# aask1357/hilcodec

Hardware: AMD Instinct MI355X
Metric: audio-seconds/sec (xRT) encode+RVQ+decode, 24 kHz batch=256 (higher is better)
Workload: dtype f32

## Files before the change

### hilcodec_amd/csrc/resblock_kernel.h

```cpp
#pragma once
#include "resblock_gemm.h"
#include "stream_gemm.h"

namespace {

struct Cols {
  long b;
  int t;
  int t_in;
  unsigned boff;
  unsigned hoff;
  int head, tail;
};
static_assert(sizeof(Cols) == 32, "no padding");

template <int C, bool STREAM, bool SCARRY = false, int NB = 1, bool W8 = false, int DRU = 0, bool POST = false, bool SPEC0 = false>
__global__ __launch_bounds__((Cfg<C, STREAM, SCARRY, NB, W8, DRU, POST, SPEC0>::NT), (Cfg<C, STREAM, SCARRY, NB, W8, DRU, POST, SPEC0>::MINW)) void resblock_kernel(ResArgs a) {
  using K = Cfg<C, STREAM, SCARRY, NB, W8, DRU, POST, SPEC0>;
  constexpr int DR = K::DR, UR = K::UR;
  using Pipe = WeightPipe<K>;
  constexpr int CBW = K::CBW, NW = K::NW, NT = K::NT, RW = K::RW, RB = K::RB, XS = K::XS, TO = K::TO, RSTEP = K::RSTEP;
  __shared__ __attribute__((aligned(16))) float Xbuf[4 + C * XS];
  constexpr bool DW_RELOAD = NB > 1 && K::NARROW && (4 + C * XS + NB * C * DWS) * 4 > 156 * 1024;
  __shared__ __attribute__((aligned(16))) float DW[(DW_RELOAD ? 1 : NB) * C * DWS];
  constexpr bool DWIDE = DR == 5 || DR == 8;
  __shared__ __attribute__((aligned(16))) float DWD[(DR > 0 && !DWIDE) ? 2 * C * DDS : 4];
  __shared__ __attribute__((aligned(16))) float HS[(STREAM && !K::NARROW) ? 2 * C * 4 : 4];
  __shared__ __attribute__((aligned(16))) float PR[POST ? POST_CLASSES * K::NCOL : 4];
  static_assert(!POST || (K::RPI * K::NW == POST_CLASSES), "a row class of the closing conv = the rows one half-wave walks");
  __shared__ __attribute__((aligned(16))) float SEG[SPEC0 ? (STREAM ? 256 : 192) : 4];
  __shared__ __attribute__((aligned(16))) float SEGS[SPEC0 ? (STREAM ? 256 : 192) : 4];
  float* const X = Xbuf + 4;
  const int tid = threadIdx.x, lane = tid & 63;
  const int wave = __builtin_amdgcn_readfirstlane(tid >> 6);
  constexpr int NCB = K::NCOL / 32;
  const int colblk = wave % NCB;
  const int wclass = wave / NCB;
  const int rowblk0 = wclass * CBW;
#if defined(HILC_DEBUG_WAVE_STAMPS)
  constexpr int WS_MAXB = 48;
  unsigned long long* ws_base = nullptr;
  int ws_k = 0;
#define STAMP(i) do { } while (0)
#define lds_barrier() do {                                                                                          \
    const unsigned long long t0_ = __builtin_amdgcn_s_memtime();                                                   \
    asm volatile("s_waitcnt lgkmcnt(0)" ::: "memory");                                                             \
    const unsigned long long t1_ = __builtin_amdgcn_s_memtime();                                                   \
    asm volatile("s_waitcnt lgkmcnt(0)\n\ts_barrier" ::: "memory");                                                 \
    const unsigned long long t2_ = __builtin_amdgcn_s_memtime();                                                   \
    if (ws_base != nullptr && lane == 0 && ws_k < WS_MAXB - 1) {                                                   \
      ws_base[ws_k * 3] = t0_; ws_base[ws_k * 3 + 1] = t1_; ws_base[ws_k * 3 + 2] = t2_;                           \
    }                                                                                                              \
    ++ws_k;                                                                                                        \
  } while (0)
#elif defined(HILC_DEBUG_STAMPS)
#define STAMP(i) do { if (a.dbg && tid == 0) a.dbg[stamp_tile * 8 + (i)] = __builtin_amdgcn_s_memtime(); } while (0)
  long stamp_tile = blockIdx.x;
#else
#define STAMP(i) do { } while (0)
#endif
  const int T = a.T;
  const int nblk = NB == 1 ? 1 : a.nblk;
  auto load_taps = [&](const ResBlk& bq, float* dst) {
    if constexpr (DW_RELOAD && !STREAM) {
      constexpr int NE = C * DWS;
      static_assert(NE % NT == 0, "whole rounds");
#pragma unroll
      for (int i = 0; i < NE / NT; ++i) {
        const int e = tid + i * NT;
        const int m = e / DWS, j = e - m * DWS;
        const float* src = j < 5 ? bq.dw1_w + (m * 5 + j) : (j == 5 ? bq.dw1_b + m : (j < 11 ? bq.dw2_w + (m * 5 + (j - 6)) : bq.dw2_b + m));
        dst[e] = *src;
      }
    } else if constexpr (DW_RELOAD) {
      constexpr int NE = C * DWS;
      static_assert(NE % NT == 0, "whole rounds");
#pragma unroll 3
      for (int i = 0; i < NE / NT; ++i) {
        const int e = tid + i * NT;
        const int m = e / DWS, j = e - m * DWS;
        const float* src = j < 5 ? bq.dw1_w + (m * 5 + j) : (j == 5 ? bq.dw1_b + m : (j < 11 ? bq.dw2_w + (m * 5 + (j - 6)) : bq.dw2_b + m));
        dst[e] = *src;
      }
    }
  };
  if constexpr (!DW_RELOAD) {
    constexpr int RND = (C + NT - 1) / NT;
    if constexpr (NB == 1 && STREAM) {
      const ResBlk& bq = a.blk[0];
#pragma unroll
      for (int it = 0; it < RND; ++it) {
        const int m = tid + it * NT;
        const int mc = (C % NT == 0 || m < C) ? m : C - 1;
#pragma unroll
        for (int w4 = 0; w4 < DWS / 4; ++w4) {
          float t4[4];
#pragma unroll
          for (int e = 0; e < 4; ++e) {
            const int j = 4 * w4 + e;
            t4[e] = j < 5 ? bq.dw1_w[mc * 5 + j] : (j == 5 ? bq.dw1_b[mc] : (j < 11 ? bq.dw2_w[mc * 5 + (j - 6)] : bq.dw2_b[mc]));
          }
          if (C % NT == 0 || m < C) *reinterpret_cast<f32x4*>(&DW[m * DWS + 4 * w4]) = f32x4{t4[0], t4[1], t4[2], t4[3]};
          __builtin_amdgcn_sched_barrier(0);
        }
      }
    } else {
    float tv[NB][RND][DWS];
#pragma unroll
    for (int q = 0; q < NB; ++q) {
      if (q < nblk) {
        const ResBlk& bq = a.blk[q];
#pragma unroll
        for (int it = 0; it < RND; ++it) {
          const int m = tid + it * NT;
          const int mc = (C % NT == 0 || m < C) ? m : C - 1;
#pragma unroll
          for (int j = 0; j < 5; ++j) tv[q][it][j] = bq.dw1_w[mc * 5 + j];
          tv[q][it][5] = bq.dw1_b[mc];
#pragma unroll
          for (int j = 0; j < 5; ++j) tv[q][it][6 + j] = bq.dw2_w[mc * 5 + j];
          tv[q][it][11] = bq.dw2_b[mc];
        }
      }
    }
#pragma unroll
    for (int q = 0; q < NB; ++q) {
      if (q < nblk) {
#pragma unroll
        for (int it = 0; it < RND; ++it) {
          const int m = tid + it * NT;
          if (C % NT == 0 || m < C) {
#pragma unroll
            for (int w4 = 0; w4 < DWS / 4; ++w4)
              *reinterpret_cast<f32x4*>(&DW[(q * C + m) * DWS + 4 * w4]) =
                  f32x4{tv[q][it][4 * w4], tv[q][it][4 * w4 + 1], tv[q][it][4 * w4 + 2], tv[q][it][4 * w4 + 3]};
          }
        }
      }
    }
    }
  }
  if constexpr (DR > 0 && !DWIDE) {
    constexpr int RND = (2 * C + NT - 1) / NT;
    float tw[RND][2 * DR + 1];
#pragma unroll
    for (int it = 0; it < RND; ++it) {
      const int m = tid + it * NT;
      const int mc = ((2 * C) % NT == 0 || m < 2 * C) ? m : 2 * C - 1;
#pragma unroll
      for (int j = 0; j < 2 * DR; ++j) tw[it][j] = a.dn.dw_w[mc * 2 * DR + j];
      tw[it][2 * DR] = a.dn.dw_b[mc];
    }
#pragma unroll
    for (int it = 0; it < RND; ++it) {
      const int m = tid + it * NT;
      if ((2 * C) % NT == 0 || m < 2 * C) {
#pragma unroll
        for (int j = 0; j < DDS; ++j) DWD[m * DDS + j] = j < 2 * DR ? tw[it][j] : (j == 8 ? tw[it][2 * DR] : 0.f);
      }
    }
  }
  if (tid < 4) Xbuf[tid] = 0.f;
  const int rsub = wave * K::RPI + (K::RPI > 1 ? lane / (K::NCOL / 4) : 0);
  const int c4 = (lane & (K::NCOL / 4 - 1)) * 4;
  [[maybe_unused]] const unsigned row_b = (unsigned)T * 4u;
  [[maybe_unused]] const bool one_head = STREAM && !K::NARROW && T >= K::NCOL;

  auto columns_of = [&](long tile) -> Cols {
    Cols s;
    s.boff = 0; s.hoff = 0; s.head = false; s.tail = false;
    if constexpr (STREAM) {
      const int flat = (int)tile * TO - K::HALO + c4;
      s.t_in = flat >= 0 && flat < a.B * T;
      const unsigned ub = s.t_in ? __umulhi((unsigned)flat, a.div_magic) >> a.div_shift : 0u;
      s.b = ub;
      s.t = s.t_in ? flat - (int)ub * T : 0;
      s.boff = (ub * (unsigned)(C * T) + (unsigned)s.t) * 4u;
      s.hoff = ub * (unsigned)(C * 4);
      s.head = s.t_in && s.t == 0;
      s.tail = s.t_in && c4 >= K::HALO && s.t == T - 4;
    } else {
      s.b = tile / a.tiles;
      s.t = (int)(tile - s.b * a.tiles) * TO + c4;
      s.t_in = s.t >= 0 && s.t < T;
    }
    return s;
  };
  auto xrow = [&](const Cols& s, int m) -> const f32x4* {
    if constexpr (STREAM)
      return reinterpret_cast<const f32x4*>(reinterpret_cast<const char*>(a.x) + (s.boff + (unsigned)m * row_b));
    else
      return reinterpret_cast<const f32x4*>(a.x + s.b * (long)C * T + (long)m * T + (s.t_in ? s.t : 0));
  };
  auto yrow = [&](const Cols& s, int m) -> f32x4* {
    if constexpr (STREAM)
      return reinterpret_cast<f32x4*>(reinterpret_cast<char*>(a.y) + (s.boff + (unsigned)m * row_b));
    else
      return reinterpret_cast<f32x4*>(a.y + s.b * (long)C * T + (long)m * T + s.t);
  };

  [[maybe_unused]] const float* hb0 = a.x;
  [[maybe_unused]] const float* hb1 = a.x;
  [[maybe_unused]] bool hv0 = false, hv1 = false;
  [[maybe_unused]] int blk_off = 0;
  Cols cs;
  const bool lane0 = c4 == 0, lane_last = c4 == K::NCOL - 4;
  auto prev_base = [&](int which) -> lptr_t {
    if constexpr (!K::CARRYMODE) return (lptr_t)(X + rsub * XS + c4 - 4);
    else return lane0 ? (lptr_t)(X + rsub * XS + K::NCOL + which * 4 + blk_off) : (lptr_t)(X + rsub * XS + c4 - 4);
  };
  auto prevs_of = [&](lptr_t pb, int m0, int which, f32x4 (&prev)[K::RB]) {
    if constexpr (!STREAM) {
#pragma unroll
      for (int i = 0; i < K::RB; ++i) prev[i] = *(lvec_t)(pb + i * RSTEP * XS);
    } else {
      bool staged = false;
      if constexpr (!K::NARROW) staged = one_head;
      if (staged) {
#pragma unroll
        for (int i = 0; i < K::RB; ++i) {
          const lptr_t pa = cs.head ? (lptr_t)(HS + (which * C + m0 + RSTEP * i) * 4) : pb + i * RSTEP * XS;
          prev[i] = *(lvec_t)pa;
        }
      } else {
        f32x4 hv[K::RB];
#pragma unroll
        for (int i = 0; i < K::RB; ++i)
          hv[i] = *reinterpret_cast<const f32x4*>((which ? hb1 : hb0) + ((which ? hv1 : hv0) ? cs.hoff + (unsigned)(m0 + RSTEP * i) * 4u : 0u));
#pragma unroll
        for (int i = 0; i < K::RB; ++i) {
          const f32x4 own = *(lvec_t)(pb + i * RSTEP * XS);
#pragma unroll
          for (int e = 0; e < 4; ++e) prev[i][e] = cs.head ? ((which ? hv1 : hv0) ? hv[i][e] : 0.f) : own[e];
        }
      }
    }
  };
  auto carry_out = [&](lptr_t xp, int which, const f32x4 (&cur)[K::RB]) {
    if constexpr (K::CARRYMODE) {
      if (lane_last) {
#pragma unroll
        for (int i = 0; i < K::RB; ++i) *(lvec_t)(xp + i * RSTEP * XS + 4 + which * 4 + blk_off) = cur[i];
      }
    }
  };

  float touch = 0.f;
  constexpr int LPR = K::NCOL / 32;
#ifdef HILC_RES_NO_UTOUCH
  constexpr bool UTOUCH = false;
#else
  constexpr bool UTOUCH = !STREAM && UR > 0 && !K::NARROW && (K::NCOL / (UR > 0 ? UR : 1)) % 32 == 0;
#endif
  constexpr int LPRU = UTOUCH ? K::NCOL / UR / 32 : 1;
  constexpr int NTOUCH = STREAM ? 1 : (UTOUCH ? (2 * C * LPRU + NT - 1) / NT : (C * LPR + NT - 1) / NT);
  float tv[NTOUCH];
#pragma unroll
  for (int i = 0; i < NTOUCH; ++i) tv[i] = 0.f;
  __shared__ long s_next;
  long run0 = blockIdx.x, run1 = a.total_tiles;
  long tile = blockIdx.x;
  if constexpr (K::CARRYMODE) {
    if (a.classes > 1) {
      const unsigned P = gridDim.x / (unsigned)a.classes, u = blockIdx.x % P, c = blockIdx.x / P;
      const long s0 = (long)u * a.total_tiles / P, len = (long)(u + 1) * a.total_tiles / P - s0;
      run0 = s0 + ((len * (long)a.cum[c]) >> 16);
      run1 = s0 + ((len * (long)a.cum[c + 1]) >> 16);
    } else if (a.run_tiles > 0) {
      run0 = (long)blockIdx.x * a.run_tiles;
      run1 = run0 + a.run_tiles < a.total_tiles ? run0 + a.run_tiles : a.total_tiles;
    } else {
      run0 = (long)blockIdx.x * a.total_tiles / gridDim.x;
      run1 = ((long)blockIdx.x + 1) * a.total_tiles / gridDim.x;
    }
    const bool mid = STREAM ? (run0 * TO) % T != 0 : run0 % a.tiles != 0;
    tile = (mid && run0 < run1) ? run0 - 1 : run0;
  }
  cs = columns_of(tile < run1 ? tile : 0);
  f32x4 xr[RW];
  if (UR == 0 && !SPEC0 && tile < run1) {
#pragma unroll
    for (int i = 0; i < RW; ++i) xr[i] = *xrow(cs, rsub + RSTEP * i);
  }
  lds_barrier();
  while (tile < run1) {
    const bool warm = K::CARRYMODE && tile < run0;
    constexpr bool TICKETS = !K::CARRYMODE && K::NW == 4;
    if constexpr (K::CARRYMODE && !STREAM) {
      if (tile % a.tiles == 0) {
        constexpr int NSLOT = 2 * NB + K::DCAR / 2 + (POST ? 1 : 0);
        for (int e = tid; e < NSLOT * C; e += NT)
          *reinterpret_cast<f32x4*>(X + (e / NSLOT) * XS + K::NCOL + (e % NSLOT) * 4) = f32x4{0.f, 0.f, 0.f, 0.f};
      }
    }
    if constexpr (!K::CARRYMODE) {
      if (TICKETS && a.sched != nullptr && tid == 0) s_next = (long)gridDim.x + atomicAdd(a.sched, 1);
    }
#if defined(HILC_DEBUG_WAVE_STAMPS)
    if (a.dbg != nullptr) {
      if (ws_base != nullptr && lane == 0) ws_base[(WS_MAXB - 1) * 3 + 1] = (unsigned long long)ws_k;
      ws_base = a.dbg + ((tile * NW + wave) * (long)WS_MAXB) * 3;
      if (lane == 0) { ws_base[(WS_MAXB - 1) * 3] = blockIdx.x; ws_base[(WS_MAXB - 1) * 3 + 2] = __builtin_amdgcn_s_memtime(); }
    }
    ws_k = 0;
#elif defined(HILC_DEBUG_STAMPS)
    stamp_tile = tile;
#endif
    STAMP(0);
    long next_tile = K::CARRYMODE ? tile + 1 : tile + gridDim.x;
    if constexpr (UR > 0) {
      const ResUp& up = a.up;
      const int Tin = T / UR;
      const int q0 = cs.t / UR, p0 = cs.t - q0 * UR;
      f32x16 acc[CBW];
#pragma unroll
      for (int i = 0; i < CBW; ++i)
#pragma unroll
        for (int r = 0; r < 16; ++r) acc[i][r] = 0.f;
#pragma nounroll
      for (int h = 0; h < 2; ++h) {
        const float* wu = (h ? up.w_hi : up.w_lo) + (long)wclass * (C * C / K::RH);
        asm volatile("" : "+s"(wu));
        {
          constexpr int UB = RW % 6 == 0 ? 6 : RB;
          constexpr bool UEXP = UR == 5;
          lptr_t xp = (lptr_t)(X + rsub * XS + c4);
          const bool has_prev = cs.t_in && q0 >= 1;
          [[maybe_unused]] const bool has_next = cs.t_in && q0 + 1 < Tin;
#pragma unroll
          for (int i0 = 0; i0 < RW; i0 += UB) {
            float xc[UB], xq[UB];
            [[maybe_unused]] float xn[UB];
            f32x4 wa[UB];
            [[maybe_unused]] f32x4 wb[UB];
#pragma unroll
            for (int i = 0; i < UB; ++i) {
              const int k = h * C + rsub + RSTEP * (i0 + i);
              const long row = (long)cs.b * (2 * C) + k;
              const float* xi = up.xin + (cs.t_in ? row * Tin + q0 : 0);
              xc[i] = xi[0];
              const float* pp = has_prev ? xi - 1 : (up.hist != nullptr && cs.t_in ? up.hist + row : xi);
              xq[i] = pp[0];
              if constexpr (UR == 2) {
                xn[i] = xi[cs.t_in ? 1 : 0];
                wa[i] = *reinterpret_cast<const f32x4*>(up.tr_w + k * 4);
              } else if constexpr (UEXP) {
                xn[i] = xi[has_next ? 1 : 0];
                const float* tw = up.tr_w + ((long)k * UR + p0) * 8;
                wa[i] = *reinterpret_cast<const f32x4*>(tw);
                wb[i] = *reinterpret_cast<const f32x4*>(tw + 4);
              } else {
                wa[i] = *reinterpret_cast<const f32x4*>(up.tr_w + k * (2 * UR) + p0);
                wb[i] = *reinterpret_cast<const f32x4*>(up.tr_w + k * (2 * UR) + UR + p0);
              }
            }
#pragma unroll
            for (int i = 0; i < UB; ++i) {
              const float a1 = prologue(xc[i], up.in_scale, 1);
              const float a0 = has_prev ? prologue(xq[i], up.in_scale, 1) : (up.hist != nullptr ? xq[i] : 0.f);
              f32x4 u;
              float a_last = a1;
              if constexpr (UR == 2) {
                const float a2 = prologue(xn[i], up.in_scale, 1);
                u[0] = fmaf(wa[i].x, a1, wa[i].z * a0);
                u[1] = fmaf(wa[i].y, a1, wa[i].w * a0);
                u[2] = fmaf(wa[i].x, a2, wa[i].z * a1);
                u[3] = fmaf(wa[i].y, a2, wa[i].w * a1);
                a_last = a2;
              } else if constexpr (UEXP) {
                const float a2 = has_next ? prologue(xn[i], up.in_scale, 1) : 0.f;
#pragma unroll
                for (int e = 0; e < 4; ++e) {
                  const bool nx = p0 + e >= UR;
                  u[e] = fmaf(wa[i][e], nx ? a2 : a1, wb[i][e] * (nx ? a1 : a0));
                }
                a_last = p0 + 3 >= UR ? a2 : a1;
              } else {
#pragma unroll
                for (int e = 0; e < 4; ++e) u[e] = fmaf(wa[i][e], a1, wb[i][e] * a0);
              }
              *(lvec_t)(xp + i * RSTEP * XS) = zero_unless(cs.t_in, u);
              if constexpr (STREAM) {
                if (cs.tail && !warm && up.hist_out != nullptr)
                  up.hist_out[(long)cs.b * (2 * C) + h * C + rsub + RSTEP * (i0 + i)] = a_last;
              }
            }
            xp += UB * RSTEP * XS;
            asm volatile("" : "+v"(xp));
            __builtin_amdgcn_sched_barrier(0);
          }
        }
        Pipe wp;
        wp.prefetch(wu, lane);
        lds_barrier();
        if constexpr (K::NARROW) gemm_phase_rolled<K, false>(wu, X, acc, wp, colblk, lane);
        else gemm_phase<K, false>(wu, X, acc, wp, colblk, lane);
        lds_barrier();
      }
      acc_to_x<K>(acc, X, rowblk0, colblk, lane);
      lds_barrier();
      {
        lptr_t xp = (lptr_t)(X + rsub * XS + c4);
#pragma unroll
        for (int i = 0; i < RW; ++i) {
          const float bv = up.bias != nullptr ? up.bias[rsub + RSTEP * i] : 0.f;
          f32x4 v = *(lvec_t)(xp + i * RSTEP * XS);
#pragma unroll
          for (int e = 0; e < 4; ++e) v[e] = up.bias != nullptr ? __fadd_rn(v[e], bv) : v[e];
          xr[i] = v;
        }
      }
      lds_barrier();
    }
    if constexpr (SPEC0) {
      const ResSpec0& sp = a.spec;
      constexpr int N = 64, NBIN = 33, SROWS = 40, KP0 = 4, DEPTH0 = 2;
      [[maybe_unused]] int split = K::NCOL;
      if constexpr (STREAM) {
        const int F0 = (int)tile * TO;
        const unsigned bA = __umulhi((unsigned)F0, a.div_magic) >> a.div_shift;
        const int tA0 = F0 - (int)bA * T;
        const int nxt = T - tA0;
        split = nxt < K::NCOL ? nxt : K::NCOL;
        const int lenA = (N - 1) + split;
        for (int i = tid; i < 2 * (N - 1) + K::NCOL; i += NT) {
          const bool second = i >= lenA;
          const unsigned b = bA + (second ? 1u : 0u);
          const int t = second ? i - lenA - (N - 1) : tA0 - (N - 1) + i;
          float v = 0.f;
          if (b < (unsigned)a.B) {
            if (t >= 0) v = sp.wav[(long)b * T + t];
            else if (sp.hist != nullptr && t >= -sp.hist_len) v = sp.hist[(long)b * sp.hist_len + sp.hist_len + t];
          }
          SEG[i] = v;
          SEGS[i] = v * sp.pre_in_scale;
        }
        for (int i = tid; i < (SROWS - NBIN) * 128; i += NT) X[(NBIN + (i >> 7)) * XS + (i & 127)] = 0.f;
      } else {
      const int f0 = cs.t - c4;
      {
        const int s0 = f0 - (N - 1);
        const float* wb = sp.wav + cs.b * (long)T;
        for (int i = tid; i < 127 + N; i += NT) {
          const int t = s0 + i;
          const float v = (t >= 0 && t < T) ? wb[t] : 0.f;
          SEG[i] = v;
          SEGS[i] = v * sp.pre_in_scale;
        }
        for (int i = tid; i < (SROWS - NBIN) * 128; i += NT) X[(NBIN + (i >> 7)) * XS + (i & 127)] = 0.f;
      }
      }
      lds_barrier();
      const int kh = lane >> 5, col = colblk * 32 + (lane & 31);
      const int colx = col + ((STREAM && col >= split) ? N - 1 : 0);
      f32x16 acc[CBW];
      {
        int off[8];
#pragma unroll
        for (int p = 0; p < 8; ++p) off[p] = colx + 2 * p + kh;
        auto bop = [&](int P) -> float { return SEG[off[P & 7] + 16 * (P >> 3)]; };
        stream_gemm<CBW, KP0, DEPTH0, N / 2 / KP0>(sp.dft, acc, lane, bop);
      }
      float nyq_im = 0.f;
#pragma unroll 8
      for (int k = 0; k < N; ++k) nyq_im = fmaf(sp.nyq[k], SEG[colx + k], nyq_im);
      const SpecFinish finish = SpecFinish::make(sp.mean, sp.stdv, sp.normalize);
#pragma unroll
      for (int i = 0; i < CBW; ++i) {
#pragma unroll
        for (int r = 0; r < 16; r += 2) {
          const int row = i * 32 + acc_row(r, lane);
          if (i == 0 && r == 0) {
            if (kh == 0) {
              X[0 * XS + col] = finish(acc[0][0], 0.f);
              X[(N / 2) * XS + col] = finish(acc[0][1], nyq_im);
            } else {
              X[(row >> 1) * XS + col] = finish(acc[0][0], acc[0][1]);
            }
          } else {
            X[(row >> 1) * XS + col] = finish(acc[i][r], acc[i][r + 1]);
          }
        }
      }
      lds_barrier();
      {
        const float* sl = X + kh * XS + col;
        auto bop = [&](int P) -> float { return sl[2 * P * XS]; };
        stream_gemm<CBW, KP0, DEPTH0, SROWS / 2 / KP0>(sp.pw, acc, lane, bop);
      }
      lds_barrier();
      acc_to_x<K>(acc, X, rowblk0, colblk, lane);
      lds_barrier();
      {
        lptr_t xp = (lptr_t)(X + rsub * XS + c4);
        float sm[8];
        const int c4x = c4 + ((STREAM && c4 >= split) ? N - 1 : 0);
#pragma unroll
        for (int j = 0; j < 8; ++j) sm[j] = SEGS[c4x + j + N - 5];
#pragma unroll
        for (int i = 0; i < RW; ++i) {
          const int m = rsub + RSTEP * i;
          const float bv = sp.bias != nullptr ? sp.bias[m] : 0.f;
          const float pb = sp.pre_b != nullptr ? sp.pre_b[m] : 0.f;
          float w5[5];
#pragma unroll
          for (int j = 0; j < 5; ++j) w5[j] = sp.pre_w[m * 5 + j];
          f32x4 v = *(lvec_t)(xp + i * RSTEP * XS);
#pragma unroll
          for (int e = 0; e < 4; ++e) {
            float acc5 = 0.f;
#pragma unroll
            for (int j = 0; j < 5; ++j) acc5 = fmaf(w5[j], sm[e + j], acc5);
            const float rr = sp.pre_b != nullptr ? __fadd_rn(acc5, pb) : acc5;
            float t = v[e];
            if (sp.bias != nullptr) t = __fadd_rn(t, bv);
            t = __fmul_rn(t, sp.out_scale);
            v[e] = __fadd_rn(t, rr);
          }
          xr[i] = v;
          if (i % 2 == 1) __builtin_amdgcn_sched_barrier(0);
        }
      }
      lds_barrier();
    }
#pragma nounroll
    for (int blk = 0; blk < nblk; ++blk) {
    const ResBlk& bp = a.blk[NB == 1 ? 0 : blk];
    const bool final_blk = NB == 1 || blk == nblk - 1;
    const bool last_blk = DR == 0 && !POST && final_blk;
    [[maybe_unused]] const bool post_blk = POST && final_blk;
    Cols cn = cs;
    bool have_next = false;
    if constexpr (NB > 1) blk_off = 8 * blk;
    const float* const DWb = DW + ((NB == 1 || DW_RELOAD) ? 0 : blk * C * DWS);
    if constexpr (DW_RELOAD) load_taps(bp, DW);
    if constexpr (STREAM) {
      hb0 = bp.hist1 != nullptr ? bp.hist1 : a.x;
      hb1 = bp.hist2 != nullptr ? bp.hist2 : a.x;
      hv0 = bp.hist1 != nullptr;
      hv1 = bp.hist2 != nullptr;
    }
    const float* w1t = bp.w1t + (long)wclass * (C * C / K::RH);
    const float* w2t = bp.w2t + (long)wclass * (C * C / K::RH);
    asm volatile("" : "+s"(w1t), "+s"(w2t));
    [[maybe_unused]] f32x4 hstage[(STREAM && !K::NARROW) ? (2 * C + NT - 1) / NT : 1];
    [[maybe_unused]] bool stage_hs = false;
    if constexpr (STREAM && !K::NARROW) {
      if (one_head) {
        const int first = (int)tile * TO - K::HALO, last = first + K::NCOL - 1;
        const unsigned bh = __umulhi((unsigned)last, a.div_magic) >> a.div_shift;
        const int hcol = (int)bh * T;
        stage_hs = hcol >= first && (int)bh < a.B;
        if (stage_hs) {
#pragma unroll
          for (int q = 0; q < (2 * C + NT - 1) / NT; ++q) {
            const int e = tid + q * NT;
            const int which = e >= C ? 1 : 0, m = e - which * C;
            f32x4 v = {0.f, 0.f, 0.f, 0.f};
            if (e < 2 * C && (which ? hv1 : hv0)) v = *reinterpret_cast<const f32x4*>((which ? hb1 : hb0) + bh * (unsigned)(C * 4) + (unsigned)m * 4u);
            hstage[q] = v;
          }
        }
      }
    }
    Pipe wp;
    wp.prefetch(w1t, lane);
    {
      lptr_t xp = (lptr_t)(X + rsub * XS + c4);
#pragma unroll
      for (int i0 = 0; i0 < RW; i0 += RB) {
#pragma unroll
        for (int i = 0; i < RB; ++i)
          *(lvec_t)(xp + i * RSTEP * XS) = prologue4v(zero_unless(cs.t_in, xr[i0 + i]), bp.pre_scale, 1);
        xp += RB * RSTEP * XS;
        asm volatile("" : "+v"(xp));
      }
    }
#pragma unroll
    for (int i = 0; i < NTOUCH; ++i) touch += tv[i];
    if constexpr (STREAM && !K::NARROW) {
      if (stage_hs) {
#pragma unroll
        for (int q = 0; q < (2 * C + NT - 1) / NT; ++q) {
          const int e = tid + q * NT;
          if (e < 2 * C) *reinterpret_cast<f32x4*>(&HS[e * 4]) = hstage[q];
        }
      }
    }
    lds_barrier();
    STAMP(1);
    if (TICKETS && a.sched != nullptr) next_tile = s_next;

    f32x16 acc[CBW];
    if constexpr (K::NARROW) gemm_phase_rolled<K>(w1t, X, acc, wp, colblk, lane);
    else gemm_phase<K>(w1t, X, acc, wp, colblk, lane);
    lds_barrier();
    STAMP(2);
    acc_to_x<K>(acc, X, rowblk0, colblk, lane);
    lds_barrier();
    STAMP(3);

    wp.prefetch(w2t, lane);
    lptr_t xp3 = (lptr_t)(X + rsub * XS + c4);
    lptr_t pb3 = prev_base(0);
#pragma unroll
    for (int i0 = 0; i0 < RW; i0 += RB) {
      f32x4 cur[RB], prev[RB], wa[RB];
      f32x2 wb[RB];
#pragma unroll
      for (int i = 0; i < RB; ++i) {
        const int m = rsub + RSTEP * (i0 + i);
        const lptr_t row = xp3 + i * RSTEP * XS;
        cur[i] = *(lvec_t)(row);
        wa[i] = *reinterpret_cast<const f32x4*>(&DWb[m * DWS]);
        wb[i] = *reinterpret_cast<const f32x2*>(&DWb[m * DWS + 4]);
      }
      prevs_of(pb3, rsub + RSTEP * i0, 0, prev);
      carry_out(xp3, 0, cur);
      if constexpr (STREAM) {
        if (cs.tail && !warm && bp.hist1_out != nullptr) {
#pragma unroll
          for (int i = 0; i < RB; ++i)
            *reinterpret_cast<f32x4*>(bp.hist1_out + cs.hoff + (rsub + RSTEP * (i0 + i)) * 4) = cur[i];
        }
      }
      f32x4 o[RB];
#pragma unroll
      for (int i = 0; i < RB; ++i) {
        const float v[8] = {prev[i].x, prev[i].y, prev[i].z, prev[i].w, cur[i].x, cur[i].y, cur[i].z, cur[i].w};
        const float w[5] = {wa[i].x, wa[i].y, wa[i].z, wa[i].w, wb[i].x};
#pragma unroll
        for (int e = 0; e < 4; ++e) {
          float s = 0.f;
#pragma unroll
          for (int j = 0; j < 5; ++j) s = fmaf(w[j], v[e + j], s);
          o[i][e] = elu_fast(__fadd_rn(s, wb[i].y));
        }
      }
#pragma unroll
      for (int i = 0; i < RB; ++i)
        *(lvec_t)(xp3 + i * RSTEP * XS) = o[i];
      xp3 += RB * RSTEP * XS;
      pb3 += RB * RSTEP * XS;
      asm volatile("" : "+v"(xp3), "+v"(pb3));
      __builtin_amdgcn_sched_barrier(0);
    }
    lds_barrier();
    STAMP(4);

    if constexpr (K::NARROW) gemm_phase_rolled<K>(w2t, X, acc, wp, colblk, lane);
    else gemm_phase<K>(w2t, X, acc, wp, colblk, lane);
    have_next = next_tile < run1;
    if (last_blk) cn = columns_of(have_next ? next_tile : tile);
    if constexpr (!STREAM && UR == 0 && !SPEC0) {
      if (final_blk) {
      long nb;
      int nt0;
      if constexpr (STREAM) {
        const int nf0 = (int)(have_next ? next_tile : tile) * TO - K::HALO;
        const unsigned q = __umulhi((unsigned)(nf0 < 0 ? 0 : nf0), a.div_magic) >> a.div_shift;
        nb = q;
        nt0 = nf0 - (int)q * T;
      } else {
        const long nt = have_next ? next_tile : tile;
        nb = nt / a.tiles;
        nt0 = (int)(nt - nb * a.tiles) * TO;
      }
      const float* nx = a.x + nb * (long)C * T;
#pragma unroll
      for (int i = 0; i < NTOUCH; ++i) {
        int e = tid + NT * i;
        e = e < C * LPR ? e : C * LPR - 1;
        int tt = nt0 + (e % LPR) * 32;
        tt = tt < 0 ? 0 : (tt > T - 1 ? T - 1 : tt);
        tv[i] = nx[(long)(e / LPR) * T + tt];
      }
      }
    }
    if constexpr (UTOUCH) {
      if (final_blk) {
        const long nt = have_next ? next_tile : tile;
        const long nb = nt / a.tiles;
        const int Tin = T / UR;
        const int nq0 = (int)(nt - nb * a.tiles) * TO / UR;
        const float* nx = a.up.xin + nb * (long)(2 * C) * Tin;
#pragma unroll
        for (int i = 0; i < NTOUCH; ++i) {
          int e = tid + NT * i;
          e = e < 2 * C * LPRU ? e : 2 * C * LPRU - 1;
          int ff = nq0 + (e % LPRU) * 32;
          ff = ff > Tin - 1 ? Tin - 1 : ff;
          tv[i] = nx[(long)(e / LPRU) * Tin + ff];
        }
      }
    }
    lds_barrier();
    STAMP(5);
    acc_to_x<K>(acc, X, rowblk0, colblk, lane);
    lds_barrier();
    STAMP(6);

    const bool out_ok = !warm && (STREAM ? (c4 >= K::HALO && cs.t_in) : cs.t < T);
    lptr_t xp6 = (lptr_t)(X + rsub * XS + c4);
    lptr_t pb6 = prev_base(1);
#pragma unroll
    for (int i0 = 0; i0 < RW; i0 += RB) {
      f32x4 cur[RB], prev[RB], wc[RB];
      f32x2 wb[RB];
#pragma unroll
      for (int i = 0; i < RB; ++i) {
        const int m = rsub + RSTEP * (i0 + i);
        const lptr_t row = xp6 + i * RSTEP * XS;
        cur[i] = *(lvec_t)(row);
        wb[i] = *reinterpret_cast<const f32x2*>(&DWb[m * DWS + 6]);
        wc[i] = *reinterpret_cast<const f32x4*>(&DWb[m * DWS + 8]);
      }
      prevs_of(pb6, rsub + RSTEP * i0, 1, prev);
      carry_out(xp6, 1, cur);
      if constexpr (STREAM) {
        if (cs.tail && !warm && bp.hist2_out != nullptr) {
#pragma unroll
          for (int i = 0; i < RB; ++i)
            *reinterpret_cast<f32x4*>(bp.hist2_out + cs.hoff + (rsub + RSTEP * (i0 + i)) * 4) = cur[i];
        }
      }
#pragma unroll
      for (int i = 0; i < RB; ++i) {
        const int m = rsub + RSTEP * (i0 + i);
        const float v[8] = {prev[i].x, prev[i].y, prev[i].z, prev[i].w, cur[i].x, cur[i].y, cur[i].z, cur[i].w};
        const float w[5] = {wb[i].x, wb[i].y, wc[i].x, wc[i].y, wc[i].z};
        f32x4 o;
#pragma unroll
        for (int e = 0; e < 4; ++e) {
          float s = 0.f;
#pragma unroll
          for (int j = 0; j < 5; ++j) s = fmaf(w[j], v[e + j], s);
          s = __fmul_rn(__fadd_rn(s, wc[i].w), bp.out_scale);
          o[e] = __fadd_rn(s, xr[i0 + i][e]);
        }
        if constexpr (NB == 1 && DR == 0 && !POST) {
          if (out_ok) *yrow(cs, m) = o;
        } else {
          if (last_blk) {
            if (out_ok) *yrow(cs, m) = o;
          } else if (post_blk) {
            *(lvec_t)(xp6 + i * RSTEP * XS) = prologue4v(o, a.post.in_scale, 1);
          } else {
            xr[i0 + i] = o;
          }
        }
      }
      if (UR == 0 && !SPEC0 && last_blk && have_next) {
#pragma unroll
        for (int i = 0; i < RB; ++i) xr[i0 + i] = *xrow(cn, rsub + RSTEP * (i0 + i));
      }
      xp6 += RB * RSTEP * XS;
      pb6 += RB * RSTEP * XS;
      asm volatile("" : "+v"(xp6), "+v"(pb6));
      __builtin_amdgcn_sched_barrier(0);
    }
    STAMP(7);
    lds_barrier();
    if (last_blk) cs = cn;
    }
    if constexpr (POST) {
      const bool have_next = next_tile < run1;
      const Cols cn = columns_of(have_next ? next_tile : tile);
      constexpr int PSLOT = K::NCOL + 8 * NB;
      float part[4] = {0.f, 0.f, 0.f, 0.f};
      lptr_t xq = (lptr_t)(X + rsub * XS + c4);
      lptr_t pq = lane0 ? (lptr_t)(X + rsub * XS + PSLOT) : (lptr_t)(X + rsub * XS + c4 - 4);
      const float* wq = a.post.w + rsub * 5;
      [[maybe_unused]] bool any_head = false;
      [[maybe_unused]] const float* hq = a.post.w;
      [[maybe_unused]] float* hqo = nullptr;
      [[maybe_unused]] bool qtail = false;
      if constexpr (STREAM) {
        const int first = (int)tile * TO, last = first + K::NCOL - 1;
        const unsigned bl = __umulhi((unsigned)last, a.div_magic) >> a.div_shift;
        any_head = (int)bl * T >= first || first % T == 0;
        if (a.post.hist != nullptr) hq = a.post.hist + cs.hoff + rsub * 4;
        qtail = cs.tail && !warm && a.post.hist_out != nullptr;
        if (a.post.hist_out != nullptr) hqo = a.post.hist_out + cs.hoff + rsub * 4;
      }
#pragma nounroll
      for (int i0 = 0; i0 < RW; i0 += RB) {
        f32x4 cur[RB], prev[RB];
        float w[RB][5];
#pragma unroll
        for (int i = 0; i < RB; ++i) {
          cur[i] = *(lvec_t)(xq + i * RSTEP * XS);
          prev[i] = *(lvec_t)(pq + i * RSTEP * XS);
#pragma unroll
          for (int j = 0; j < 5; ++j) w[i][j] = wq[i * RSTEP * 5 + j];
        }
        wq += RB * RSTEP * 5;
        if constexpr (STREAM) {
          if (any_head) {
            f32x4 hv[RB];
#pragma unroll
            for (int i = 0; i < RB; ++i)
              hv[i] = a.post.hist != nullptr ? *reinterpret_cast<const f32x4*>(hq + i * RSTEP * 4) : f32x4{0.f, 0.f, 0.f, 0.f};
#pragma unroll
            for (int i = 0; i < RB; ++i)
#pragma unroll
              for (int e = 0; e < 4; ++e) prev[i][e] = cs.head ? hv[i][e] : prev[i][e];
          }
          if (qtail) {
#pragma unroll
            for (int i = 0; i < RB; ++i) *reinterpret_cast<f32x4*>(hqo + i * RSTEP * 4) = cur[i];
          }
          hq += a.post.hist != nullptr ? RB * RSTEP * 4 : 0;
          hqo += RB * RSTEP * 4;
        }
        if (lane_last) {
#pragma unroll
          for (int i = 0; i < RB; ++i) *(lvec_t)(xq + i * RSTEP * XS + 4 + 8 * NB) = cur[i];
        }
#pragma unroll
        for (int i = 0; i < RB; ++i) {
          const float v[8] = {prev[i].x, prev[i].y, prev[i].z, prev[i].w, cur[i].x, cur[i].y, cur[i].z, cur[i].w};
#pragma unroll
          for (int e = 0; e < 4; ++e)
#pragma unroll
            for (int j = 0; j < 5; ++j) part[e] = fmaf(w[i][j], v[e + j], part[e]);
        }
        xq += RB * RSTEP * XS;
        pq += RB * RSTEP * XS;
        asm volatile("" : "+v"(xq), "+v"(pq));
        __builtin_amdgcn_sched_barrier(0);
      }
      *reinterpret_cast<f32x4*>(&PR[rsub * K::NCOL + c4]) = f32x4{part[0], part[1], part[2], part[3]};
      lds_barrier();
      if (tid < K::NCOL) {
        float sacc = PR[tid];
#pragma unroll
        for (int q = 1; q < POST_CLASSES; ++q) sacc = __fadd_rn(sacc, PR[q * K::NCOL + tid]);
        if (a.post.bias != nullptr) sacc = __fadd_rn(sacc, a.post.bias[0]);
        sacc = __fmul_rn(sacc, a.post.out_scale);
        if (a.post.do_tanh) sacc = tanhf(sacc);
        if constexpr (STREAM) {
          const long flat = (long)tile * TO + tid;
          if (!warm && flat < (long)a.B * T) a.post.wav[flat] = sacc;
        } else {
          const int t = cs.t - c4 + tid;
          if (!warm && t < T) a.post.wav[cs.b * (long)T + t] = sacc;
        }
      }
      cs = cn;
    }
    if constexpr (DR > 0) {
      const ResDown& dn = a.dn;
      const bool have_next = next_tile < run1;
      const Cols cn = columns_of(have_next ? next_tile : tile);
      const float* wd0 = dn.w_lo + (long)wclass * (C * C / K::RH);
      const float* wd1 = dn.w_hi + (long)wclass * (C * C / K::RH);
      asm volatile("" : "+s"(wd0), "+s"(wd1));
      Pipe wp;
      wp.prefetch(wd0, lane);
      auto d0 = [&]() {
        lptr_t xp = (lptr_t)(X + rsub * XS + c4);
#pragma unroll
        for (int i0 = 0; i0 < RW; i0 += RB) {
#pragma unroll
          for (int i = 0; i < RB; ++i)
            *(lvec_t)(xp + i * RSTEP * XS) = prologue4v(zero_unless(cs.t_in, xr[i0 + i]), dn.in_scale, 1);
          xp += RB * RSTEP * XS;
          asm volatile("" : "+v"(xp));
        }
      };
      d0();
      if (!DWIDE && !SPEC0 && have_next) {
#pragma unroll
        for (int i = 0; i < RW; ++i) xr[i] = *xrow(cn, rsub + RSTEP * i);
      }
      lds_barrier();
      f32x16 acc0[CBW];
      [[maybe_unused]] f32x16 acc1[DWIDE ? 1 : CBW];
      if constexpr (K::NARROW) gemm_phase_rolled<K>(wd0, X, acc0, wp, colblk, lane);
      else gemm_phase<K>(wd0, X, acc0, wp, colblk, lane);
      if constexpr (!DWIDE) {
        wp.prefetch(wd1, lane);
        if constexpr (K::NARROW) gemm_phase_rolled<K>(wd1, X, acc1, wp, colblk, lane);
        else gemm_phase<K>(wd1, X, acc1, wp, colblk, lane);
      }
      const bool out_ok = !warm && (STREAM ? cs.t_in : cs.t < T);
      [[maybe_unused]] const bool out_ok_tile = !warm;
      const int To = T / DR;
#pragma unroll
      for (int h = 0; h < 2; ++h) {
        if constexpr (DWIDE) {
          if (h == 1) {
            lds_barrier();
            wp.prefetch(wd1, lane);
            d0();
            if (have_next) {
#pragma unroll
              for (int i = 0; i < RW; ++i) xr[i] = *xrow(cn, rsub + RSTEP * i);
            }
            lds_barrier();
            gemm_phase_rolled<K>(wd1, X, acc0, wp, colblk, lane);
          }
        }
        lds_barrier();
        if constexpr (DWIDE) acc_to_x<K>(acc0, X, rowblk0, colblk, lane);
        else acc_to_x<K>(h ? acc1 : acc0, X, rowblk0, colblk, lane);
        lds_barrier();
        if constexpr (DWIDE) {
          constexpr int DC = K::DCAR;
          constexpr int DOFF = K::NCOL + 8 * NB;
          constexpr bool SLOTS = K::CARRYMODE;
          const int jl = c4 >> 2;
          const int t0 = STREAM ? (int)tile * TO : cs.t - c4;
          const int o = t0 / DR + jl;
          const int base = o * DR - DR - t0;
          [[maybe_unused]] unsigned sb = 0;
          int os = o;
          if constexpr (STREAM) {
            const bool in = o < a.B * To;
            sb = in ? __umulhi((unsigned)(o * DR), a.div_magic) >> a.div_shift : 0u;
            os = in ? o - (int)sb * To : 1;
          }
          [[maybe_unused]] const bool dhead = STREAM && os == 0;
          const bool act = out_ok_tile && (STREAM ? o < a.B * To : o < To) && o * DR + DR - 1 < t0 + K::NCOL;
          [[maybe_unused]] const int slot = DOFF + DC * h + DC;
          lptr_t rowp = (lptr_t)(X + rsub * XS);
          const float* wrow = dn.dw_w + (long)(h * C + rsub) * (2 * DR);
          const float* brow = dn.dw_b + (h * C + rsub);
          float wn[2 * DR], bn;
          [[maybe_unused]] float hn[STREAM ? DR : 1];
          [[maybe_unused]] const float* hrow = dn.dw_w;
          [[maybe_unused]] float* horow = nullptr;
          [[maybe_unused]] const bool use_hist = STREAM && dn.hist != nullptr;
          if constexpr (STREAM) {
            if (use_hist) hrow = dn.hist + ((long)sb * (2 * C) + h * C + rsub) * DR;
            if (dn.hist_out != nullptr) horow = dn.hist_out + ((long)cs.b * (2 * C) + h * C + rsub) * DR;
          }
          [[maybe_unused]] const bool dtail = STREAM && cs.tail && !warm && dn.hist_out != nullptr;
          auto taps_of = [&](const float* wr, const float* br) {
            if constexpr (DR == 8) {
#pragma unroll
              for (int q = 0; q < 4; ++q) {
                const f32x4 w4 = *reinterpret_cast<const f32x4*>(wr + 4 * q);
#pragma unroll
                for (int e = 0; e < 4; ++e) wn[4 * q + e] = w4[e];
              }
            } else {
#pragma unroll
              for (int q = 0; q < DR; ++q) {
                const f32x2 w2 = *reinterpret_cast<const f32x2*>(wr + 2 * q);
                wn[2 * q] = w2.x; wn[2 * q + 1] = w2.y;
              }
            }
            bn = br[0];
            if constexpr (STREAM) {
              if (use_hist) {
                if constexpr (DR == 8) {
#pragma unroll
                  for (int q = 0; q < 2; ++q) {
                    const f32x4 h4 = *reinterpret_cast<const f32x4*>(hrow + 4 * q);
#pragma unroll
                    for (int e = 0; e < 4; ++e) hn[4 * q + e] = h4[e];
                  }
                } else {
#pragma unroll
                  for (int j = 0; j < DR; ++j) hn[j] = hrow[j];
                }
              } else {
#pragma unroll
                for (int j = 0; j < DR; ++j) hn[j] = 0.f;
              }
            }
          };
          taps_of(wrow, brow);
          long yo = STREAM ? ((long)sb * (2 * C) + h * C + rsub) * (long)To + os : ((long)cs.b * (2 * C) + h * C + rsub) * (long)To + o;
#pragma nounroll
          for (int i0 = 0; i0 < RW; ++i0) {
            float v[2 * DR], w[2 * DR];
#pragma unroll
            for (int j = 0; j < 2 * DR; ++j) w[j] = wn[j];
            const float bb = bn;
            [[maybe_unused]] float hc[STREAM ? DR : 1];
            if constexpr (STREAM) {
#pragma unroll
              for (int j = 0; j < DR; ++j) hc[j] = hn[j];
            }
            wrow += RSTEP * (2 * DR);
            brow += RSTEP;
            if constexpr (STREAM) hrow += use_hist ? RSTEP * DR : 0;
            if (i0 + 1 < RW) taps_of(wrow, brow);
            if constexpr (DR == 8) {
#pragma unroll
              for (int q = 0; q < 4; ++q) {
                const int col = base + 4 * q;
                const f32x4 x4 = *(lvec_t)(rowp + (col >= 0 ? col : (SLOTS ? slot + col : 0)));
#pragma unroll
                for (int e = 0; e < 4; ++e) v[4 * q + e] = x4[e];
              }
            } else {
#pragma unroll
              for (int j = 0; j < 2 * DR; ++j) {
                const int col = base + j;
                v[j] = *(rowp + (col >= 0 ? col : (SLOTS ? slot + col : 0)));
              }
            }
            if constexpr (STREAM) {
#pragma unroll
              for (int j = 0; j < DR; ++j) v[j] = dhead ? hc[j] : v[j];
            }
            const f32x4 keep = *(lvec_t)(rowp + c4);
            if constexpr (STREAM) {
              const f32x4 before = *(lvec_t)(rowp + (c4 >= 4 ? c4 - 4 : 0));
              if (dtail) {
                if constexpr (DR == 8) {
                  *reinterpret_cast<f32x4*>(horow) = before;
                  *reinterpret_cast<f32x4*>(horow + 4) = keep;
                } else {
                  horow[0] = before.w; horow[1] = keep.x; horow[2] = keep.y; horow[3] = keep.z; horow[4] = keep.w;
                }
              }
              horow += RSTEP * DR;
            }
            if constexpr (SLOTS) {
              if (c4 >= K::NCOL - DC)
                *(lvec_t)(rowp + DOFF + DC * h + (c4 - (K::NCOL - DC))) = keep;
            }
            float s0 = 0.f;
#pragma unroll
            for (int j = 0; j < 2 * DR; ++j) s0 = fmaf(w[j], v[j], s0);
            s0 = __fadd_rn(s0, bb);
            if (act) dn.y[yo] = dn.res != nullptr ? __fadd_rn(s0, dn.res[yo]) : s0;
            yo += (long)RSTEP * To;
            rowp += RSTEP * XS;
          }
        } else {
        lptr_t xpd = (lptr_t)(X + rsub * XS + c4);
        lptr_t pbd = lane0 ? (lptr_t)(X + rsub * XS + K::NCOL + 8 * NB + 4 * h) : (lptr_t)(X + rsub * XS + c4 - 4);
#pragma unroll
        for (int i0 = 0; i0 < RW; i0 += RB) {
          f32x4 cur[RB], prev[RB], wa[RB], wb[RB];
          float bb[RB];
#pragma unroll
          for (int i = 0; i < RB; ++i) {
            const int m = h * C + rsub + RSTEP * (i0 + i);
            cur[i] = *(lvec_t)(xpd + i * RSTEP * XS);
            prev[i] = *(lvec_t)(pbd + i * RSTEP * XS);
            wa[i] = *reinterpret_cast<const f32x4*>(&DWD[m * DDS]);
            if constexpr (DR == 4) wb[i] = *reinterpret_cast<const f32x4*>(&DWD[m * DDS + 4]);
            bb[i] = DWD[m * DDS + 8];
          }
          if constexpr (STREAM) {
            const unsigned hro = (unsigned)cs.b * (unsigned)(2 * C * DR) + (unsigned)(h * C + rsub + RSTEP * i0) * DR;
#pragma unroll
            for (int i = 0; i < RB; ++i) {
              f32x4 hv = {0.f, 0.f, 0.f, 0.f};
              if (dn.hist != nullptr) {
                const float* hp = dn.hist + (cs.t_in ? hro + (unsigned)(RSTEP * i * DR) : 0u);
                if constexpr (DR == 4) hv = *reinterpret_cast<const f32x4*>(hp);
                else { const f32x2 h2 = *reinterpret_cast<const f32x2*>(hp); hv = f32x4{0.f, 0.f, h2.x, h2.y}; }
              }
#pragma unroll
              for (int e = 0; e < 4; ++e) prev[i][e] = cs.head ? hv[e] : prev[i][e];
            }
          }
          if (lane_last) {
#pragma unroll
            for (int i = 0; i < RB; ++i) *(lvec_t)(xpd + i * RSTEP * XS + 4 + 8 * NB + 4 * h) = cur[i];
          }
          if constexpr (STREAM) {
            if (cs.tail && !warm && dn.hist_out != nullptr) {
              const unsigned hro = (unsigned)cs.b * (unsigned)(2 * C * DR) + (unsigned)(h * C + rsub + RSTEP * i0) * DR;
#pragma unroll
              for (int i = 0; i < RB; ++i) {
                float* hp = dn.hist_out + hro + (unsigned)(RSTEP * i * DR);
                if constexpr (DR == 4) *reinterpret_cast<f32x4*>(hp) = cur[i];
                else *reinterpret_cast<f32x2*>(hp) = f32x2{cur[i].z, cur[i].w};
              }
            }
          }
#pragma unroll
          for (int i = 0; i < RB; ++i) {
            const int m = h * C + rsub + RSTEP * (i0 + i);
            const long yo = ((long)cs.b * (2 * C) + m) * (long)To + (cs.t_in ? cs.t / DR : 0);
            if constexpr (DR == 4) {
              const float v[8] = {prev[i].x, prev[i].y, prev[i].z, prev[i].w, cur[i].x, cur[i].y, cur[i].z, cur[i].w};
              const float w[8] = {wa[i].x, wa[i].y, wa[i].z, wa[i].w, wb[i].x, wb[i].y, wb[i].z, wb[i].w};
              float s0 = 0.f;
#pragma unroll
              for (int j = 0; j < 8; ++j) s0 = fmaf(w[j], v[j], s0);
              s0 = __fadd_rn(s0, bb[i]);
              if (out_ok) dn.y[yo] = dn.res != nullptr ? __fadd_rn(s0, dn.res[yo]) : s0;
            } else {
              const float v[6] = {prev[i].z, prev[i].w, cur[i].x, cur[i].y, cur[i].z, cur[i].w};
              const float w[4] = {wa[i].x, wa[i].y, wa[i].z, wa[i].w};
              f32x2 o2;
#pragma unroll
              for (int e = 0; e < 2; ++e) {
                float s0 = 0.f;
#pragma unroll
                for (int j = 0; j < 4; ++j) s0 = fmaf(w[j], v[2 * e + j], s0);
                o2[e] = __fadd_rn(s0, bb[i]);
              }
              if (out_ok) {
                if (dn.res != nullptr) {
                  const f32x2 r2 = *reinterpret_cast<const f32x2*>(dn.res + yo);
                  o2[0] = __fadd_rn(o2[0], r2.x);
                  o2[1] = __fadd_rn(o2[1], r2.y);
                }
                *reinterpret_cast<f32x2*>(dn.y + yo) = o2;
              }
            }
          }
          xpd += RB * RSTEP * XS;
          pbd += RB * RSTEP * XS;
          asm volatile("" : "+v"(xpd), "+v"(pbd));
          __builtin_amdgcn_sched_barrier(0);
        }
        }
      }
      lds_barrier();
      cs = cn;
    }
    tile = next_tile;
  }
  if (!K::CARRYMODE && K::NW == 4 && a.sched != nullptr && tid == 0) {
    if (atomicAdd(a.sched + 1, 1) == (int)gridDim.x - 1) {
      a.sched[0] = 0;
      a.sched[1] = 0;
    }
  }
  if (touch == 1.2345678e-30f) a.y[0] = touch;
#if defined(HILC_DEBUG_WAVE_STAMPS)
  if (ws_base != nullptr && lane == 0) ws_base[(WS_MAXB - 1) * 3 + 1] = (unsigned long long)ws_k;
#undef lds_barrier
#endif
#undef STAMP
}

}
```

Baseline: 3528.

## Stage upsample taps in LDS and prefetch upsample inputs into registers early

For non-stream upsampling resblocks with UR 2 or 4, the transposed-conv taps are copied once into shared memory. The input frames for the next tile and next half are fetched into registers ahead of use, overlapping with the previous GEMM phase. Neighbouring frames are exchanged with DPP lane shifts instead of being read again from global memory. A separate wide-UR path using ds_bpermute is added, but its prefetch variant sits behind a macro that is off by default. The changes cost extra shared memory and register pressure and add more complex index logic.

```diff
diff --git a/hilcodec_amd/csrc/resblock_kernel.h b/hilcodec_amd/csrc/resblock_kernel.h
--- a/hilcodec_amd/csrc/resblock_kernel.h
+++ b/hilcodec_amd/csrc/resblock_kernel.h
@@ -30,6 +30,13 @@
   static_assert(!POST || (K::RPI * K::NW == POST_CLASSES), "a row class of the closing conv = the rows one half-wave walks");
   __shared__ __attribute__((aligned(16))) float SEG[SPEC0 ? (STREAM ? 256 : 192) : 4];
   __shared__ __attribute__((aligned(16))) float SEGS[SPEC0 ? (STREAM ? 256 : 192) : 4];
+  constexpr bool UFAST = !STREAM && (UR == 4 || UR == 2) && !K::NARROW;
+  __shared__ __attribute__((aligned(16))) float UT[UFAST ? 2 * C * 2 * UR : 4];
+  constexpr bool UWIDE = !STREAM && (UR == 5 || UR == 8) && K::NARROW;
+#ifndef HILC_RES_UPRE_WIDE
+#define HILC_RES_UPRE_WIDE 0
+#endif
+  constexpr bool UPRE = UFAST || (UWIDE && HILC_RES_UPRE_WIDE);
   float* const X = Xbuf + 4;
   const int tid = threadIdx.x, lane = tid & 63;
   const int wave = __builtin_amdgcn_readfirstlane(tid >> 6);
@@ -42,6 +49,7 @@
   unsigned long long* ws_base = nullptr;
   int ws_k = 0;
 #define STAMP(i) do { } while (0)
+#define USTAMP(i) do { } while (0)
 #define lds_barrier() do {                                                                                          \
     const unsigned long long t0_ = __builtin_amdgcn_s_memtime();                                                   \
     asm volatile("s_waitcnt lgkmcnt(0)" ::: "memory");                                                             \
@@ -56,8 +64,11 @@
 #elif defined(HILC_DEBUG_STAMPS)
 #define STAMP(i) do { if (a.dbg && tid == 0) a.dbg[stamp_tile * 8 + (i)] = __builtin_amdgcn_s_memtime(); } while (0)
   long stamp_tile = blockIdx.x;
+  constexpr long USTAMP_ROW0 = 1l << 19;
+#define USTAMP(i) do { if (a.dbg && tid == 0) a.dbg[(USTAMP_ROW0 + stamp_tile) * 8 + (i)] = __builtin_amdgcn_s_memtime(); } while (0)
 #else
 #define STAMP(i) do { } while (0)
+#define USTAMP(i) do { } while (0)
 #endif
   const int T = a.T;
   const int nblk = NB == 1 ? 1 : a.nblk;
@@ -158,6 +169,20 @@
 #pragma unroll
         for (int j = 0; j < DDS; ++j) DWD[m * DDS + j] = j < 2 * DR ? tw[it][j] : (j == 8 ? tw[it][2 * DR] : 0.f);
       }
+    }
+  }
+  if constexpr (UFAST) {
+    constexpr int NQ = 2 * C * 2 * UR / 4;
+    f32x4 tq[(NQ + NT - 1) / NT];
+#pragma unroll
+    for (int it = 0; it < (NQ + NT - 1) / NT; ++it) {
+      const int e = tid + it * NT;
+      tq[it] = *reinterpret_cast<const f32x4*>(a.up.tr_w + 4 * (NQ % NT == 0 || e < NQ ? e : 0));
+    }
+#pragma unroll
+    for (int it = 0; it < (NQ + NT - 1) / NT; ++it) {
+      const int e = tid + it * NT;
+      if (NQ % NT == 0 || e < NQ) *reinterpret_cast<f32x4*>(&UT[4 * e]) = tq[it];
     }
   }
   if (tid < 4) Xbuf[tid] = 0.f;
@@ -278,6 +303,35 @@
   }
   cs = columns_of(tile < run1 ? tile : 0);
   f32x4 xr[RW];
+  [[maybe_unused]] float uxl = 0.f;
+  [[maybe_unused]] auto u_request = [&](const Cols& c, int h, int i0, int n) {
+    if constexpr (UFAST || UWIDE) {
+      constexpr int LPRW = K::NCOL / 4;
+      const int Tin = T / UR;
+      const int j = lane & (LPRW - 1), hw = lane / LPRW;
+      const int qt0 = (c.t - c4) / UR;
+      const float* rowp = a.up.xin + ((long)c.b * (2 * C) + h * C + wave * K::RPI) * Tin;
+      int fq;
+      if constexpr (UFAST) fq = c.t_in ? c.t / UR : 0;
+      else fq = (qt0 - 1 + j >= 0 && qt0 - 1 + j < Tin) ? qt0 - 1 + j : 0;
+      const unsigned voff = (unsigned)(hw * Tin + fq) * 4u;
+      const int rowstep = RSTEP * Tin;
+#pragma unroll
+      for (int i = 0; i < RW; ++i) {
+        if (i >= i0 && i < i0 + n) {
+          const float* xi = reinterpret_cast<const float*>(reinterpret_cast<const char*>(rowp + (long)i * rowstep) + voff);
+          xr[i].x = xi[0];
+          if constexpr (UFAST && UR == 2) xr[i].y = xi[1];
+        }
+      }
+      if constexpr (UFAST) {
+        if (i0 == 0) uxl = rowp[(j < RW && qt0 >= 1) ? (long)(hw + RSTEP * j) * Tin + (qt0 - 1) : 0];
+      }
+    }
+  };
+  if constexpr (UPRE) {
+    if (tile < run1) u_request(cs, 0, 0, RW);
+  }
   if (UR == 0 && !SPEC0 && tile < run1) {
 #pragma unroll
     for (int i = 0; i < RW; ++i) xr[i] = *xrow(cs, rsub + RSTEP * i);
@@ -312,6 +366,7 @@
       const ResUp& up = a.up;
       const int Tin = T / UR;
       const int q0 = cs.t / UR, p0 = cs.t - q0 * UR;
+      USTAMP(0);
       f32x16 acc[CBW];
 #pragma unroll
       for (int i = 0; i < CBW; ++i)
@@ -321,7 +376,101 @@
       for (int h = 0; h < 2; ++h) {
         const float* wu = (h ? up.w_hi : up.w_lo) + (long)wclass * (C * C / K::RH);
         asm volatile("" : "+s"(wu));
-        {
+        if constexpr (UFAST) {
+          static_assert(RW <= 16 && K::NCOL == 128 && K::RPI == 2, "a half-wave = one row; the gather lives in one DPP row");
+          constexpr int UB = RW % 6 == 0 ? 6 : RB;
+          constexpr int FPL = 4 / UR;
+          const int j = lane & 31;
+          const int qt0 = (cs.t - c4) / UR;
+          float L = (j < RW && qt0 >= 1) ? prologue(uxl, up.in_scale, 1) : 0.f;
+          lptr_t xp = (lptr_t)(X + rsub * XS + c4);
+          lptr_t tp = (lptr_t)(UT + (h * C + rsub) * (2 * UR));
+#pragma unroll
+          for (int i0 = 0; i0 < RW; i0 += UB) {
+#pragma unroll
+            for (int i = 0; i < UB; ++i) {
+              float a1 = prologue(xr[i0 + i].x, up.in_scale, 1);
+              a1 = cs.t_in ? a1 : 0.f;
+              float al = a1;
+              [[maybe_unused]] float a2 = 0.f;
+              if constexpr (FPL == 2) {
+                a2 = prologue(xr[i0 + i].y, up.in_scale, 1);
+                a2 = cs.t_in ? a2 : 0.f;
+                al = a2;
+              }
+              float a0 = __int_as_float(__builtin_amdgcn_update_dpp(__float_as_int(L), __float_as_int(al), 0x138, 0xf, 0xf, false));
+              a0 = lane == 32 ? L : a0;
+              a0 = cs.t_in ? a0 : 0.f;
+              L = __int_as_float(__builtin_amdgcn_update_dpp(0, __float_as_int(L), 0x101, 0xf, 0xf, false));
+              f32x4 u;
+              if constexpr (UR == 2) {
+                const f32x4 w = *(lvec_t)(tp + (i0 + i) * RSTEP * 4);
+                u[0] = fmaf(w.x, a1, w.z * a0);
+                u[1] = fmaf(w.y, a1, w.w * a0);
+                u[2] = fmaf(w.x, a2, w.z * a1);
+                u[3] = fmaf(w.y, a2, w.w * a1);
+              } else {
+                const f32x4 wa = *(lvec_t)(tp + (i0 + i) * RSTEP * 8);
+                const f32x4 wb = *(lvec_t)(tp + (i0 + i) * RSTEP * 8 + 4);
+#pragma unroll
+                for (int e = 0; e < 4; ++e) u[e] = fmaf(wa[e], a1, wb[e] * a0);
+              }
+              *(lvec_t)(xp + i * RSTEP * XS) = u;
+            }
+            xp += UB * RSTEP * XS;
+            asm volatile("" : "+v"(xp));
+            __builtin_amdgcn_sched_barrier(0);
+          }
+        } else if constexpr (UWIDE) {
+          constexpr int LPRW = K::NCOL / 4;
+          constexpr int UB = RW % 6 == 0 ? 6 : RB;
+          constexpr bool UEXP = UR == 5;
+          static_assert((K::NCOL + UR - 1) / UR + 2 <= LPRW, "a row's lanes hold every frame its columns read");
+          const int j = lane & (LPRW - 1);
+          const int t0 = cs.t - c4;
+          const int qb = t0 / UR;
+          const int fq = qb - 1 + j;
+          const bool fv = fq >= 0 && fq < Tin;
+          const int sl = (lane & ~(LPRW - 1)) + (q0 - qb);
+          const int pa1 = sl * 4 + 4, pa0 = cs.t_in ? sl * 4 : pa1;
+          [[maybe_unused]] const int pa2 = sl * 4 + 8;
+          const float* twl = up.tr_w + (UEXP ? ((long)(h * C + rsub) * UR + p0) * 8 : (long)(h * C + rsub) * (2 * UR) + p0);
+          lptr_t xp = (lptr_t)(X + rsub * XS + c4);
+#pragma unroll
+          for (int i0 = 0; i0 < RW; i0 += UB) {
+            f32x4 wa[UB], wb[UB];
+            if constexpr (!UPRE) u_request(cs, h, i0, UB);
+#pragma unroll
+            for (int i = 0; i < UB; ++i) {
+              const float* tw = twl + (i0 + i) * (RSTEP * (UEXP ? UR * 8 : 2 * UR));
+              wa[i] = *reinterpret_cast<const f32x4*>(tw);
+              wb[i] = *reinterpret_cast<const f32x4*>(tw + (UEXP ? 4 : UR));
+            }
+#pragma unroll
+            for (int i = 0; i < UB; ++i) {
+              float av = prologue(xr[i0 + i].x, up.in_scale, 1);
+              av = fv ? av : 0.f;
+              const float a0 = __int_as_float(__builtin_amdgcn_ds_bpermute(pa0, __float_as_int(av)));
+              const float a1 = __int_as_float(__builtin_amdgcn_ds_bpermute(pa1, __float_as_int(av)));
+              f32x4 u;
+              if constexpr (UEXP) {
+                const float a2 = __int_as_float(__builtin_amdgcn_ds_bpermute(pa2, __float_as_int(av)));
+#pragma unroll
+                for (int e = 0; e < 4; ++e) {
+                  const bool nx = e > 0 && p0 + e >= UR;
+                  u[e] = fmaf(wa[i][e], nx ? a2 : a1, wb[i][e] * (nx ? a1 : a0));
+                }
+              } else {
+#pragma unroll
+                for (int e = 0; e < 4; ++e) u[e] = fmaf(wa[i][e], a1, wb[i][e] * a0);
+              }
+              *(lvec_t)(xp + i * RSTEP * XS) = u;
+            }
+            xp += UB * RSTEP * XS;
+            asm volatile("" : "+v"(xp));
+            __builtin_amdgcn_sched_barrier(0);
+          }
+        } else {
           constexpr int UB = RW % 6 == 0 ? 6 : RB;
           constexpr bool UEXP = UR == 5;
           lptr_t xp = (lptr_t)(X + rsub * XS + c4);
@@ -390,12 +539,17 @@
             __builtin_amdgcn_sched_barrier(0);
           }
         }
+        if constexpr (UPRE) {
+          if (h == 0) u_request(cs, 1, 0, RW);
+        }
         Pipe wp;
         wp.prefetch(wu, lane);
         lds_barrier();
+        USTAMP(1 + 2 * h);
         if constexpr (K::NARROW) gemm_phase_rolled<K, false>(wu, X, acc, wp, colblk, lane);
         else gemm_phase<K, false>(wu, X, acc, wp, colblk, lane);
         lds_barrier();
+        USTAMP(2 + 2 * h);
       }
       acc_to_x<K>(acc, X, rowblk0, colblk, lane);
       lds_barrier();
@@ -411,6 +565,7 @@
         }
       }
       lds_barrier();
+      USTAMP(5);
     }
     if constexpr (SPEC0) {
       const ResSpec0& sp = a.spec;
@@ -651,7 +806,7 @@
     if constexpr (K::NARROW) gemm_phase_rolled<K>(w2t, X, acc, wp, colblk, lane);
     else gemm_phase<K>(w2t, X, acc, wp, colblk, lane);
     have_next = next_tile < run1;
-    if (last_blk) cn = columns_of(have_next ? next_tile : tile);
+    if (last_blk || (UPRE && final_blk)) cn = columns_of(have_next ? next_tile : tile);
     if constexpr (!STREAM && UR == 0 && !SPEC0) {
       if (final_blk) {
       long nb;
@@ -753,6 +908,9 @@
       if (UR == 0 && !SPEC0 && last_blk && have_next) {
 #pragma unroll
         for (int i = 0; i < RB; ++i) xr[i0 + i] = *xrow(cn, rsub + RSTEP * (i0 + i));
+      }
+      if constexpr (UPRE) {
+        if (final_blk && have_next) u_request(cn, 0, i0, RB);
       }
       xp6 += RB * RSTEP * XS;
       pb6 += RB * RSTEP * XS;
@@ -1135,6 +1293,7 @@
 #undef lds_barrier
 #endif
 #undef STAMP
+#undef USTAMP
 }
 
 }
```

Result: no change. 3551 (median of 6 runs) (+0.7%).
